# AegisIK/DistMLIP

Hardware: NVIDIA H100
Metric: atoms/sec (energy+forces) CHGNet a-Si r_cut=5A (higher is better)
Workload: dtype f32

## Files before the change

### distmlip_b200/csrc/kernels.cu

```cuda
#include "final_tail.cuh"
#include "kernels.cuh"
#include "wgmma.cuh"

#include <algorithm>

namespace b2m {

__device__ __forceinline__ float sigm(float x) {
  float e, r;
  asm("ex2.approx.ftz.f32 %0, %1;" : "=f"(e) : "f"(x * -1.4426950408889634f));
  asm("rcp.approx.ftz.f32 %0, %1;" : "=f"(r) : "f"(1.f + e));
  return r;
}
__device__ __forceinline__ float silu_f(float x) { return x * sigm(x); }
__device__ __forceinline__ float dsilu_f(float x) {
  float s = sigm(x);
  return s * (1.f + x * (1.f - s));
}

__device__ __forceinline__ uint32_t smem_u32(const void* p) { return (uint32_t)__cvta_generic_to_shared(p); }
__device__ __forceinline__ void mbar_init(uint64_t* bar, uint32_t count) {
  asm volatile("mbarrier.init.shared::cta.b64 [%0], %1;" ::"r"(smem_u32(bar)), "r"(count) : "memory");
}
__device__ __forceinline__ void fence_barrier_init() {
// ... 225 lines not shown
}
__global__ void k_dsilu_mul(int64_t n, const float* __restrict__ pre, float* __restrict__ g) {
  const int64_t i = blockIdx.x * (int64_t)blockDim.x + threadIdx.x;
  if (i < n) g[i] *= dsilu_f(pre[i]);
}
void launch_silu(cudaStream_t st, int64_t n, const float* pre, float* out) {
  launch(k_silu, cdiv(n, 256), 256, 0, st, n, pre, out);
}
void launch_dsilu_mul(cudaStream_t st, int64_t n, const float* pre, float* g) {
  launch(k_dsilu_mul, cdiv(n, 256), 256, 0, st, n, pre, g);
}
void launch_zero_rows(cudaStream_t st, float* p, int64_t nfloats) {
  if (nfloats > 0) B2M_CK(cudaMemsetAsync(p, 0, nfloats * sizeof(float), st));
}

constexpr int LDE = 136;

struct EdgeRow {
  int src, dst, bond;
  float d;
};
__device__ __forceinline__ EdgeRow edge_row(const AtomConvArgs& a, int64_t e, bool has_row) {
  EdgeRow r{-1, -1, -1, 1.f};
  if (has_row && e < a.E) {
    r.src = a.e_src[e];
    r.dst = a.e_dst[e];
    r.bond = a.e_bond[e];
    r.d = a.e_vec[e].w;
  }
  return r;
}
template <int ROWS>
__device__ __forceinline__ void issue_gather(const AtomConvArgs& a, int64_t t, const EdgeRow& row, int lr, float* buf,
                                             uint64_t* bar, int* s_src, int* s_dst, int* s_bond, float* s_d) {
  if (lr == 0) mbar_expect_tx(bar, (uint32_t)min((int64_t)ROWS, a.E - t * ROWS) * 512u);
  if (lr < ROWS) {
    if (s_src != nullptr) s_src[lr] = row.src;
    s_dst[lr] = row.dst;
    s_bond[lr] = row.bond;
    s_d[lr] = row.d;
    if (row.src >= 0) bulk_g2s(buf + lr * LDE, a.Aproj + (size_t)row.src * D2, 512u, bar);
  }
}
template <int ROWS>
__device__ __forceinline__ void radial_rows(const AtomConvArgs& a, const float* s_d, int nvalid, float* be_s, float* be8,
                                            float* dbe_s, float* dbe8) {
  const int r = threadIdx.x % ROWS, half = (threadIdx.x / ROWS) & 1;
  const float d = s_d[r];
  const int k0 = half ? 5 : 0, k1 = half ? 9 : 5;
  for (int k = k0; k < k1; k++) {
    float be = 0.f, dbe = 0.f;
    if (r < nvalid) rbf_env_k(d, a.rp.freq[k], a.rp, be, dbe);
    *(k < 8 ? be_s + r * 8 + k : be8 + r) = be;
    if (dbe_s != nullptr) *(k < 8 ? dbe_s + r * 8 + k : dbe8 + r) = dbe;
  }
}
__device__ __forceinline__ float2 ld_f2(const float* p) { return *reinterpret_cast<const float2*>(p); }
__device__ __forceinline__ void st_f2(float* p, float x, float y) { *reinterpret_cast<float2*>(p) = make_float2(x, y); }

__device__ __forceinline__ constexpr int fq(int ii, int j) { return 4 * (j >> 1) + 2 * ii + (j & 1); }

__device__ __forceinline__ void radial_mma(const Map& m, int h, const float* x_s, const float* img, float (&d)[32]) {
  const float2 u = ld_f2(x_s + m.row(2 * h) * 8 + m.cb), v = ld_f2(x_s + m.row(2 * h + 1) * 8 + m.cb);
  const float x[1][4] = {{u.x, v.x, u.y, v.y}};
  uint32_t b = s_u32(img);
  asm volatile("" : "+r"(b));
  wg_mma64(x, b, b + 512u * 4u, 0, false, d);
}

template <int R>
__device__ __forceinline__ void first_layer_half(const AtomConvArgs& a, const Map& m, int h, const float* tile,
                                                 const int* s_dst, const int* s_bond, const float* be_s,
                                                 const float* be8, const float* rad, int nvalid,
                                                 float (&acc)[R][AC]) {
  const int c0 = 64 * m.branch + m.cb;
  float2 cv[2][AC / 2], qv[2][AC / 2];
  float b8[2];
  bool viaQ[2], ok[2];
#pragma unroll
  for (int ii = 0; ii < 2; ii++) {
    const int r = m.row(2 * h + ii);
    const int dst = s_dst[r], bond = s_bond[r];
    ok[ii] = r < nvalid;
    viaQ[ii] = a.Qproj != nullptr && bond >= 0;
    const float* cp = a.Cproj + (size_t)max(dst, 0) * D2 + c0;
#pragma unroll
    for (int jj = 0; jj < AC / 2; jj++) cv[ii][jj] = dst >= 0 ? __ldg(reinterpret_cast<const float2*>(cp + 8 * jj)) : make_float2(0.f, 0.f);
    if (viaQ[ii]) {
      const float* qp = a.Qproj + (size_t)bond * D2 + c0;
#pragma unroll
      for (int jj = 0; jj < AC / 2; jj++) qv[ii][jj] = __ldg(reinterpret_cast<const float2*>(qp + 8 * jj));
    } else {
#pragma unroll
      for (int jj = 0; jj < AC / 2; jj++) qv[ii][jj] = make_float2(0.f, 0.f);
    }
    b8[ii] = be8[r];
  }
  float d[32];
  radial_mma(m, h, be_s, rad + ATOM_RAD_M + 1024 * m.branch, d);
#pragma unroll
  for (int j = 0; j < AC; j++) {
    const float m8 = rad[ATOM_RAD_M8 + 64 * m.branch + m.col(j)];
#pragma unroll
    for (int ii = 0; ii < 2; ii++) {
      const int r = m.row(2 * h + ii);
      const float x = tile[r * LDE + 64 * m.branch + m.col(j)];
      const float2 c2 = cv[ii][j >> 1], q2 = qv[ii][j >> 1];
      const float t = viaQ[ii] ? ((j & 1) ? q2.y : q2.x) : fmaf(b8[ii], m8, d[fq(ii, j)]);
      acc[2 * h + ii][j] = ok[ii] ? x + ((j & 1) ? c2.y : c2.x) + t : 0.f;
    }
  }
}

template <int R>
__device__ __forceinline__ void wg_mm64_acc(const float (&x)[R][AC], int h, const float* Bcan, float (&acc)[R][AC]) {
  float v[8][4];
#pragma unroll
  for (int ks = 0; ks < 8; ks++) {
    v[ks][0] = x[2 * h][2 * ks], v[ks][1] = x[2 * h + 1][2 * ks];
    v[ks][2] = x[2 * h][2 * ks + 1], v[ks][3] = x[2 * h + 1][2 * ks + 1];
  }
  const uint32_t b_hi = s_u32(Bcan);
  float d[32];
  wg_mma64(v, b_hi, b_hi + 4096u * 4u, 0, false, d);
#pragma unroll
  for (int q = 0; q < 32; q++) acc[2 * h + ((q >> 1) & 1)][2 * (q >> 2) + (q & 1)] = d[q];
}

__device__ __forceinline__ float quad_row_sum(const float (&v)[AR]) {
  const int l = threadIdx.x & 3;
  const bool b0 = l & 1, b1 = l & 2;
  float w[2];
#pragma unroll
  for (int h = 0; h < 2; h++)
    w[h] = (b0 ? v[2 * h + 1] : v[2 * h]) + __shfl_xor_sync(0xffffffffu, b0 ? v[2 * h] : v[2 * h + 1], 1);
  return (b1 ? w[1] : w[0]) + __shfl_xor_sync(0xffffffffu, b1 ? w[0] : w[1], 2);
}

__device__ __forceinline__ void red_add_v4(float* p, float4 v) {
  asm volatile("red.global.add.v4.f32 [%0], {%1, %2, %3, %4};" ::"l"(p), "f"(v.x), "f"(v.y), "f"(v.z), "f"(v.w)
               : "memory");
}

__device__ __forceinline__ void seg_add(float* out, int width, int col, int k, const float4& v, int& cur, float4& sum) {
  if (k != cur) {
    if (cur >= 0) red_add_v4(out + (size_t)cur * width + col, sum);
    cur = k;
    sum = make_float4(0.f, 0.f, 0.f, 0.f);
  }
  if (k >= 0) sum.x += v.x, sum.y += v.y, sum.z += v.z, sum.w += v.w;
}

template <int LPR, int ROWS = TM, int NTH = NT>
__device__ __forceinline__ void scatter_rows(const float* tile, const int* key0, float* out0, const int* key1,
                                             float* out1, const int* gidx, float* gat, const int* sidx = nullptr,
                                             float* sto = nullptr) {
  constexpr int R = ROWS * LPR / NTH, W = 4 * LPR, B = 8;
  static_assert(R % B == 0 && B % 4 == 0, "batches of B rows, their indices read as int4");
  const int t = threadIdx.x % NTH, q = t % LPR, r0 = t / LPR * R;
  float4 s0 = make_float4(0.f, 0.f, 0.f, 0.f), s1 = s0;
  int c0 = -1, c1 = -1;
#pragma unroll
  for (int b = 0; b < R; b += B) {
    float4 v[B];
    int k0[B], k1[B], kg[B], ks[B];
#pragma unroll
    for (int i = 0; i < B; i++) v[i] = *reinterpret_cast<const float4*>(tile + (r0 + b + i) * LDE + 4 * q);
    auto ld_idx = [&](const int* idx, bool on, int(&k)[B]) {
#pragma unroll
      for (int i = 0; i < B; i += 4) {
        const int4 x = on ? *reinterpret_cast<const int4*>(idx + r0 + b + i) : make_int4(-1, -1, -1, -1);
        k[i] = x.x, k[i + 1] = x.y, k[i + 2] = x.z, k[i + 3] = x.w;
      }
    };
    ld_idx(key0, out0 != nullptr, k0);
    ld_idx(key1, out1 != nullptr, k1);
    ld_idx(gidx, gat != nullptr, kg);
    ld_idx(sidx, sto != nullptr, ks);
#pragma unroll
    for (int i = 0; i < B; i++) {
      if (ks[i] >= 0) *reinterpret_cast<float4*>(sto + (size_t)ks[i] * W + 4 * q) = v[i];
      if (kg[i] >= 0) red_add_v4(gat + (size_t)kg[i] * W + 4 * q, v[i]);
      seg_add(out0, W, 4 * q, k0[i], v[i], c0, s0);
      seg_add(out1, W, 4 * q, k1[i], v[i], c1, s1);
    }
  }
  if (c0 >= 0) red_add_v4(out0 + (size_t)c0 * W + 4 * q, s0);
  if (c1 >= 0) red_add_v4(out1 + (size_t)c1 * W + 4 * q, s1);
}

constexpr int TW = 64;
constexpr int WGF = 3, NTF = 128 * WGF;
struct AtomSmemFwd {
  static constexpr int kTile = 32;
  static constexpr int kW = kTile + WGF * TW * LDE;
  static constexpr int kRad = kW + 16384;
  static constexpr int kBe = kRad + ATOM_RAD;
  static constexpr int kBe8 = kBe + WGF * TW * 8;
  static constexpr int kB2 = kBe8 + WGF * TW;
  static constexpr int kD = kB2 + 128;
  static constexpr int kIdx = kD + WGF * TW;
  static constexpr int kTotal = kIdx + 2 * WGF * TW;
  static constexpr size_t bytes = (size_t)kTotal * 4;
};
static_assert(AtomSmemFwd::bytes <= 232448, "atom-conv forward shared memory");
static_assert(AtomSmemFwd::kW % 4 == 0 && AtomSmemFwd::kRad % 4 == 0 && AtomSmemFwd::kBe % 4 == 0 &&
                  AtomSmemFwd::kIdx % 4 == 0,
              "16-byte aligned images, radial rows and index slots");

__device__ __forceinline__ void wg_sync(int w) { asm volatile("bar.sync %0, 128;" ::"r"(1 + w) : "memory"); }

__global__ void __launch_bounds__(NTF, 1) k_atomconv_fwd(const AtomConvArgs a) {
  extern __shared__ __align__(128) float smem[];
  const int tid = threadIdx.x, w = tid >> 7, lr = tid & 127;
  uint64_t* mbar = reinterpret_cast<uint64_t*>(smem) + w;
  const float* Wsm = smem + AtomSmemFwd::kW;
  const float* rad = smem + AtomSmemFwd::kRad;
  const float* b2s = smem + AtomSmemFwd::kB2;
  float* tile = smem + AtomSmemFwd::kTile + w * TW * LDE;
  float* be_s = smem + AtomSmemFwd::kBe + w * TW * 8;
  float* be8 = smem + AtomSmemFwd::kBe8 + w * TW;
  float* s_d = smem + AtomSmemFwd::kD + w * TW;
  int* s_dst = reinterpret_cast<int*>(smem + AtomSmemFwd::kIdx) + w * TW;
  int* s_bond = reinterpret_cast<int*>(smem + AtomSmemFwd::kIdx) + (WGF + w) * TW;

  const int64_t ntiles = (a.E + TW - 1) / TW, first = WGF * (int64_t)blockIdx.x + w, step = WGF * (int64_t)gridDim.x;
  if (tid == 0) {
    for (int i = 0; i < WGF; i++) mbar_init(reinterpret_cast<uint64_t*>(smem) + i, 1);
    fence_barrier_init();
  }
  EdgeRow nxt = edge_row(a, first * TW + lr, lr < TW);
  stage_w<NTF>(smem + AtomSmemFwd::kW, a.W2can, 4096);
  stage_w<NTF>(smem + AtomSmemFwd::kRad, a.radial, ATOM_RAD / 4);
  if (tid < 128) smem[AtomSmemFwd::kB2 + tid] = a.b2[tid];
  __syncthreads();
  if (first < ntiles)
    issue_gather<TW>(a, first, nxt, lr, tile, mbar, nullptr, s_dst, s_bond, s_d);
  nxt = edge_row(a, (first + step) * TW + lr, lr < TW);

  const Map m;
  Map mL = m, mG = m;
  mL.branch = 0;
  mG.branch = 1;
  int it = 0;
  for (int64_t t = first; t < ntiles; t += step, it++) {
    const int nvalid = (int)min((int64_t)TW, a.E - t * TW);
    wg_sync(w);
    radial_rows<TW>(a, s_d, nvalid, be_s, be8, nullptr, nullptr);
    mbar_wait(mbar, (uint32_t)it & 1u);
    wg_sync(w);
    float L[2][AC];
    first_layer_half(a, mL, 0, tile, s_dst, s_bond, be_s, be8, rad, nvalid, L);
#pragma unroll
    for (int ii = 0; ii < 2; ii++)
#pragma unroll
      for (int j = 0; j < AC; j++) L[ii][j] = silu_f(L[ii][j]);
    wg_mm64_acc(L, 0, Wsm, L);
#pragma unroll
    for (int ii = 0; ii < 2; ii++)
#pragma unroll
      for (int j = 0; j < AC; j++) L[ii][j] = silu_f(L[ii][j] + b2s[m.col(j)]);
    float G[2][AC];
    first_layer_half(a, mG, 0, tile, s_dst, s_bond, be_s, be8, rad, nvalid, G);
#pragma unroll
    for (int ii = 0; ii < 2; ii++)
#pragma unroll
      for (int j = 0; j < AC; j++) G[ii][j] = silu_f(G[ii][j]);
    wg_mm64_acc(G, 0, Wsm + 8192, G);
    float wab[32];
    radial_mma(m, 0, be_s, rad + ATOM_RAD_WAB, wab);
#pragma unroll
    for (int ii = 0; ii < 2; ii++) {
      const int r = m.row(ii);
      const float b8 = be8[r];
      float mv[AC];
#pragma unroll
      for (int j = 0; j < AC; j++) {
        const float g = sigm(G[ii][j] + b2s[64 + m.col(j)]) * fmaf(b8, rad[ATOM_RAD_WAB8 + m.col(j)], wab[fq(ii, j)]);
        mv[j] = L[ii][j] * g;
      }
#pragma unroll
      for (int jj = 0; jj < AC / 2; jj++) st_f2(tile + r * LDE + m.col(2 * jj), mv[2 * jj], mv[2 * jj + 1]);
    }
    wg_sync(w);
    scatter_rows<16, TW, 128>(tile, s_dst, a.agg, nullptr, nullptr, nullptr, nullptr);
    fence_proxy_async_smem();
    wg_sync(w);
    if (t + step < ntiles) {
      issue_gather<TW>(a, t + step, nxt, lr, tile, mbar, nullptr, s_dst, s_bond, s_d);
      nxt = edge_row(a, (t + 2 * step) * TW + lr, lr < TW);
    }
  }
}

void launch_atomconv_fwd(cudaStream_t st, const AtomConvArgs& a, int num_sms) {
  if (a.E <= 0) return;
  static PerDeviceOnce attr;
  if (auto once_ = attr.first(); once_) {
    B2M_CK(cudaFuncSetAttribute(k_atomconv_fwd, cudaFuncAttributeMaxDynamicSharedMemorySize, (int)AtomSmemFwd::bytes));
  }
  launch(k_atomconv_fwd, std::min(cdiv(cdiv(a.E, TW), WGF), num_sms), NTF, AtomSmemFwd::bytes, st, a);
}

struct AtomSmemBwd {
  static constexpr int kBuf = 32;
  static constexpr int kW = kBuf + 2 * TM * LDE;
  static constexpr int kRad = kW + 16384;
  static constexpr int kBe = kRad + ATOM_RAD;
  static constexpr int kDbe = kBe + TM * 8;
  static constexpr int kBe8 = kDbe + TM * 8;
  static constexpr int kDbe8 = kBe8 + TM;
  static constexpr int kB2 = kDbe8 + TM;
  static constexpr int kD = kB2 + 128;
  static constexpr int kIdx = kD + 2 * TM;
  static constexpr int kTotal = kIdx + 6 * TM;
  static constexpr size_t bytes = (size_t)kTotal * 4;
};
static_assert(AtomSmemBwd::bytes <= 232448, "atom-conv backward shared memory");
static_assert(AtomSmemBwd::kW % 4 == 0 && AtomSmemBwd::kRad % 4 == 0 && AtomSmemBwd::kBe % 4 == 0 &&
                  AtomSmemBwd::kDbe % 4 == 0,
              "16-byte aligned images and radial rows");

__global__ void __launch_bounds__(NT, 1) k_atomconv_bwd(const AtomConvArgs a) {
  extern __shared__ __align__(128) float smem[];
  uint64_t* gbar = reinterpret_cast<uint64_t*>(smem);
  uint64_t* wbar = gbar + 2;
  float* Wsm = smem + AtomSmemBwd::kW;
  float* rad_base = smem + AtomSmemBwd::kRad;
  float* be_s = smem + AtomSmemBwd::kBe;
  float* dbe_s = smem + AtomSmemBwd::kDbe;
  float* be8 = smem + AtomSmemBwd::kBe8;
  float* dbe8 = smem + AtomSmemBwd::kDbe8;
  float* b2s = smem + AtomSmemBwd::kB2;

  const int tid = threadIdx.x;
  const int64_t ntiles = (a.E + TM - 1) / TM, step = gridDim.x;
  const bool useQ = a.Qproj != nullptr;
  auto buf_of = [&](int s) { return smem + AtomSmemBwd::kBuf + s * TM * LDE; };
  auto d_of = [&](int s) { return smem + AtomSmemBwd::kD + s * TM; };
  auto src_of = [&](int s) { return reinterpret_cast<int*>(smem + AtomSmemBwd::kIdx) + s * TM; };
  auto dst_of = [&](int s) { return reinterpret_cast<int*>(smem + AtomSmemBwd::kIdx) + (2 + s) * TM; };
  auto bond_of = [&](int s) { return reinterpret_cast<int*>(smem + AtomSmemBwd::kIdx) + (4 + s) * TM; };

  if (tid == 0) {
    mbar_init(&gbar[0], 1);
    mbar_init(&gbar[1], 1);
    mbar_init(wbar, 1);
    fence_barrier_init();
  }
  EdgeRow nxt = edge_row(a, (int64_t)blockIdx.x * TM + tid, threadIdx.x < TM);
  stage_w(rad_base, a.radial, ATOM_RAD / 4);
  if (tid < 128) b2s[tid] = a.b2[tid];
  __syncthreads();
  if (tid == 0) bulk_g2s_image(Wsm, a.W2can, 16384 * 4, wbar);
  issue_gather<TM>(a, blockIdx.x, nxt, tid, buf_of(0), &gbar[0], src_of(0), dst_of(0), bond_of(0), d_of(0));
  nxt = edge_row(a, ((int64_t)blockIdx.x + step) * TM + tid, threadIdx.x < TM);
  uint32_t wpar = 0;

  const Map m;
  const int c0 = 64 * m.branch;
  int it = 0;
  for (int64_t t = blockIdx.x; t < ntiles; t += step, it++) {
    float* rad = rad_base;
    asm volatile("" : "+l"(rad));
    const int s = it & 1;
    float* tileP = buf_of(s);
    float* tileH = buf_of(s ^ 1);
    const int* s_src = src_of(s);
    const int* s_dst = dst_of(s);
    const int* s_bond = bond_of(s);
    const int64_t e0 = t * TM;
    const int nvalid = (int)min((int64_t)TM, a.E - e0);
    __syncthreads();
    radial_rows<TM>(a, d_of(s), nvalid, be_s, be8, dbe_s, dbe8);
    mbar_wait(&gbar[s], stage_parity(it));
    mbar_wait(wbar, wpar);
    wpar ^= 1;
    __syncthreads();
    float acc[AR][AC];
#pragma unroll
    for (int h = 0; h < 2; h++) {
      first_layer_half(a, m, h, tileP, s_dst, s_bond, be_s, be8, rad, nvalid, acc);
#pragma unroll
      for (int ii = 0; ii < 2; ii++)
#pragma unroll
        for (int jj = 0; jj < AC / 2; jj++) {
          float* p = tileP + m.row(2 * h + ii) * LDE + c0 + m.col(2 * jj);
          float& x0 = acc[2 * h + ii][2 * jj];
          float& x1 = acc[2 * h + ii][2 * jj + 1];
          st_f2(p, x0, x1);
          x0 = silu_f(x0);
          x1 = silu_f(x1);
        }
      wg_mm64_acc(acc, h, Wsm + m.branch * 8192, acc);
#pragma unroll
      for (int ii = 0; ii < 2; ii++)
#pragma unroll
        for (int jj = 0; jj < AC / 2; jj++) {
          const float u0 = acc[2 * h + ii][2 * jj] + b2s[m.branch * 64 + m.col(2 * jj)];
          const float u1 = acc[2 * h + ii][2 * jj + 1] + b2s[m.branch * 64 + m.col(2 * jj + 1)];
          st_f2(tileH + m.row(2 * h + ii) * LDE + c0 + m.col(2 * jj), m.branch == 0 ? u0 : sigm(u0),
                m.branch == 0 ? u1 : sigm(u1));
        }
    }
    __syncthreads();
    if (tid == 0) bulk_g2s_image(Wsm, a.W2Tcan, 16384 * 4, wbar);
    float sd[AR];
#pragma unroll
    for (int h = 0; h < 2; h++) {
      int dst[2];
      float2 gm2[2][AC / 2];
#pragma unroll
      for (int ii = 0; ii < 2; ii++) {
        dst[ii] = s_dst[m.row(2 * h + ii)];
        const float* gp = a.gagg + (size_t)max(dst[ii], 0) * D + m.cb;
#pragma unroll
        for (int jj = 0; jj < AC / 2; jj++)
          gm2[ii][jj] = dst[ii] >= 0 ? __ldg(reinterpret_cast<const float2*>(gp + 8 * jj)) : make_float2(0.f, 0.f);
      }
      float w[32];
      radial_mma(m, h, be_s, rad + ATOM_RAD_WAB, w);
#pragma unroll
      for (int ii = 0; ii < 2; ii++) {
        const int i = 2 * h + ii;
        const int r = m.row(i);
        const float b8 = be8[r];
#pragma unroll
        for (int jj = 0; jj < AC / 2; jj++) {
          const float2 ow2 = ld_f2(tileH + r * LDE + c0 + m.col(2 * jj));
          const float2 pt2 = ld_f2(tileH + r * LDE + (64 - c0) + m.col(2 * jj));
          const float2 wk2 = ld_f2(rad + ATOM_RAD_WAB8 + m.col(2 * jj));
#pragma unroll
          for (int e = 0; e < 2; e++) {
            const int j = 2 * jj + e;
            const float x = e ? ow2.y : ow2.x;
            const float pt = e ? pt2.y : pt2.x;
            const float gm = e ? gm2[ii][jj].y : gm2[ii][jj].x;
            const float wab = fmaf(b8, e ? wk2.y : wk2.x, w[fq(ii, j)]);
            float g = 0.f, gwv = 0.f;
            if (dst[ii] >= 0) {
              if (m.branch == 0) {
                const float sg = sigm(x);
                const float oL = x * sg;
                gwv = gm * oL * pt;
                g = gm * pt * wab * (sg * (1.f + x * (1.f - sg)));
              } else {
                const float oL = silu_f(pt);
                g = gm * oL * wab * x * (1.f - x);
              }
            }
            acc[i][j] = g;
            w[fq(ii, j)] = gwv;
          }
        }
      }
      sd[2 * h] = sd[2 * h + 1] = 0.f;
      if (m.branch == 0) {
        float dw[32];
        radial_mma(m, h, dbe_s, rad + ATOM_RAD_WAB, dw);
#pragma unroll
        for (int ii = 0; ii < 2; ii++) {
          const float db8 = dbe8[m.row(2 * h + ii)];
#pragma unroll
          for (int j = 0; j < AC; j++)
            sd[2 * h + ii] = fmaf(w[fq(ii, j)], fmaf(db8, rad[ATOM_RAD_WAB8 + m.col(j)], dw[fq(ii, j)]), sd[2 * h + ii]);
        }
      }
      if (h == 0) mbar_wait(wbar, wpar);
      wg_mm64_acc(acc, h, Wsm + m.branch * 8192, acc);
#pragma unroll
      for (int ii = 0; ii < 2; ii++)
#pragma unroll
        for (int jj = 0; jj < AC / 2; jj++) {
          float* p = tileP + m.row(2 * h + ii) * LDE + c0 + m.col(2 * jj);
          const float2 pre = ld_f2(p);
          float& x0 = acc[2 * h + ii][2 * jj];
          float& x1 = acc[2 * h + ii][2 * jj + 1];
          x0 *= dsilu_f(pre.x);
          x1 *= dsilu_f(pre.y);
          st_f2(p, x0, x1);
        }
      float dm[32];
      radial_mma(m, h, dbe_s, rad + ATOM_RAD_M + 1024 * m.branch, dm);
#pragma unroll
      for (int ii = 0; ii < 2; ii++) {
        const int r = m.row(2 * h + ii);
        const float db8 = dbe8[r];
        float s = 0.f;
#pragma unroll
        for (int jj = 0; jj < AC / 2; jj++) {
          const float2 mk = ld_f2(rad + ATOM_RAD_M8 + c0 + m.col(2 * jj));
          s = fmaf(acc[2 * h + ii][2 * jj], fmaf(db8, mk.x, dm[fq(ii, 2 * jj)]), s);
          s = fmaf(acc[2 * h + ii][2 * jj + 1], fmaf(db8, mk.y, dm[fq(ii, 2 * jj + 1)]), s);
        }
        if (r < nvalid && !(useQ && s_bond[r] >= 0)) sd[2 * h + ii] += s;
      }
    }
    wpar ^= 1;
    fence_proxy_async_smem();
    __syncthreads();
    if (t + step < ntiles) {
      if (tid == 0) bulk_g2s_image(Wsm, a.W2can, 16384 * 4, wbar);
      issue_gather<TM>(a, t + step, nxt, tid, tileH, &gbar[s ^ 1], src_of(s ^ 1), dst_of(s ^ 1), bond_of(s ^ 1), d_of(s ^ 1));
      nxt = edge_row(a, (t + 2 * step) * TM + tid, threadIdx.x < TM);
    }
    {
      const float v = quad_row_sum(sd);
      const int r = m.row(tid & 3);
      if (m.branch == 1) be8[r] = v;
      __syncthreads();
      if (m.branch == 0 && r < nvalid) a.gd[e0 + r] += v + be8[r];
    }
    scatter_rows<32>(tileP, s_dst, a.gA != nullptr ? a.gC : nullptr, nullptr, nullptr, s_src, a.gA, s_bond,
                     useQ ? a.gQ : nullptr);
  }
}

void launch_atomconv_bwd(cudaStream_t st, const AtomConvArgs& a, int num_sms) {
  if (a.E <= 0) return;
  static PerDeviceOnce attr;
  if (auto once_ = attr.first(); once_) {
    B2M_CK(cudaFuncSetAttribute(k_atomconv_bwd, cudaFuncAttributeMaxDynamicSharedMemorySize, (int)AtomSmemBwd::bytes));
  }
  launch(k_atomconv_bwd, std::min(cdiv(a.E, TM), num_sms), NT, AtomSmemBwd::bytes, st, a);
}

struct LineSmem {
  static constexpr int kBuf = 32;
  static constexpr int kW = kBuf + 2 * TM * LDE;
  static constexpr int kB2 = kW + 16384;
  static constexpr int kIdx = kB2 + 128;
  static constexpr int kTotal = kIdx + 6 * TM;
  static constexpr size_t bytes = (size_t)kTotal * 4;
};
static_assert(LineSmem::bytes <= 232448, "line-graph shared memory");

struct LineSm {
  float* smem;
  __device__ __forceinline__ uint64_t* hbar() const { return reinterpret_cast<uint64_t*>(smem); }
  __device__ __forceinline__ uint64_t* abar() const { return hbar() + 2; }
  __device__ __forceinline__ uint64_t* wbar() const { return hbar() + 4; }
  __device__ __forceinline__ float* buf(int s) const { return smem + LineSmem::kBuf + s * TM * LDE; }
  __device__ __forceinline__ float* W() const { return smem + LineSmem::kW; }
  __device__ __forceinline__ float* b2() const { return smem + LineSmem::kB2; }
  __device__ __forceinline__ int* idx(int s, int k) const {
    return reinterpret_cast<int*>(smem + LineSmem::kIdx) + (2 * k + s) * TM;
  }
};

struct AngleIdx {
  int a, b, c;
};
__device__ __forceinline__ AngleIdx angle_idx(const LineArgs& a, int64_t r) {
  AngleIdx x{-1, -1, -1};
  if (threadIdx.x < TM && r < a.A) {
    x.a = a.a_in[r];
    x.b = a.a_out[r];
    x.c = a.a_ctr[r];
  }
  return x;
}
__device__ __forceinline__ void line_issue_ha(const LineArgs& a, const LineSm& sm, int64_t t, const AngleIdx& x,
                                             float* buf, int s) {
  const int tid = threadIdx.x;
  if (tid == 0) mbar_expect_tx(&sm.hbar()[s], (uint32_t)min((int64_t)TM, a.A - t * TM) * 512u);
  if (tid < TM) {
    sm.idx(s, 0)[tid] = x.a;
    sm.idx(s, 1)[tid] = x.b;
    sm.idx(s, 2)[tid] = x.c;
    if (x.a >= 0) bulk_g2s(buf + tid * LDE, a.Ha + (size_t)x.a * D2, 512u, &sm.hbar()[s]);
  }
}
__device__ __forceinline__ void line_issue_ang(const LineArgs& a, const LineSm& sm, int64_t t, float* buf, int s) {
  const int tid = threadIdx.x;
  const int nvalid = (int)min((int64_t)TM, a.A - t * TM);
  if (tid == 0) mbar_expect_tx(&sm.abar()[s], (uint32_t)nvalid * 256u);
  if (tid < nvalid) bulk_g2s(buf + tid * LDE + 64, a.ang + (size_t)(t * TM + tid) * D, 256u, &sm.abar()[s]);
}
__device__ __forceinline__ AngleIdx line_prologue(const LineArgs& a, const LineSm& sm) {
  const int tid = threadIdx.x;
  if (tid == 0) {
    for (int i = 0; i < 5; i++) mbar_init(&sm.hbar()[i], 1);
    fence_barrier_init();
  }
  AngleIdx x = angle_idx(a, (int64_t)blockIdx.x * TM + tid);
  if (tid < 128) sm.b2()[tid] = a.b2 ? a.b2[tid] : 0.f;
  __syncthreads();
  if (tid == 0) bulk_g2s_image(sm.W(), a.Wgcan, 16384 * 4, sm.wbar());
  line_issue_ha(a, sm, blockIdx.x, x, sm.buf(0), 0);
  line_issue_ang(a, sm, blockIdx.x, sm.buf(1), 0);
  return angle_idx(a, ((int64_t)blockIdx.x + gridDim.x) * TM + tid);
}

__device__ __forceinline__ void line_first_layer(const LineArgs& a, const Map& m, const float* P, const int* s_b,
                                                 const int* s_c, int nvalid, float (&acc)[AR][AC]) {
  const int c0 = 64 * m.branch + m.cb;
#pragma unroll
  for (int i = 0; i < AR; i++) {
    const int r = m.row(i);
    const bool ok = r < nvalid;
    const float* hb = a.Hb + (size_t)(ok ? s_b[r] : 0) * D2 + c0;
    const float* xc = a.Xc + (size_t)(ok ? s_c[r] : 0) * D2 + c0;
    float2 hv[AC / 2], xv[AC / 2];
#pragma unroll
    for (int jj = 0; jj < AC / 2; jj++) {
      hv[jj] = ok ? __ldg(reinterpret_cast<const float2*>(hb + 8 * jj)) : make_float2(0.f, 0.f);
      xv[jj] = ok ? __ldg(reinterpret_cast<const float2*>(xc + 8 * jj)) : make_float2(0.f, 0.f);
    }
#pragma unroll
    for (int jj = 0; jj < AC / 2; jj++) {
      const float2 ha = ok ? ld_f2(P + r * LDE + c0 + 8 * jj) : make_float2(0.f, 0.f);
      float& x0 = acc[i][2 * jj];
      float& x1 = acc[i][2 * jj + 1];
      x0 = ok ? ha.x + x0 + hv[jj].x + xv[jj].x : 0.f;
      x1 = ok ? ha.y + x1 + hv[jj].y + xv[jj].y : 0.f;
    }
  }
}

__device__ __forceinline__ void red_add_v2(float* p, float x, float y) {
  asm volatile("red.global.add.v2.f32 [%0], {%1, %2};" ::"l"(p), "f"(x), "f"(y) : "memory");
}

template <bool HIDDEN>
__global__ void __launch_bounds__(NT, 1) k_line_fwd(const LineArgs a) {
  extern __shared__ __align__(128) float smem[];
  const LineSm sm{smem};
  const float* b2s = sm.b2();
  const int tid = threadIdx.x;
  const int64_t ntiles = (a.A + TM - 1) / TM, step = gridDim.x;
  AngleIdx nxt = line_prologue(a, sm);
  uint32_t wpar = 0;

  int it = 0;
  for (int64_t t = blockIdx.x; t < ntiles; t += step, it++) {
    const int s = it & 1;
    float* P = sm.buf(s);
    float* Q = sm.buf(s ^ 1);
    const int* s_b = sm.idx(s, 1);
    const int* s_c = sm.idx(s, 2);
    const int64_t r0 = t * TM;
    const int nvalid = (int)min((int64_t)TM, a.A - r0);
    const bool more = t + step < ntiles;
    const Map m;
    float acc[AR][AC];
    mbar_wait(&sm.abar()[s], stage_parity(it));
    mbar_wait(sm.wbar(), wpar);
    if (HIDDEN) wpar ^= 1;
    gemm64(Q, LDE, 64, sm.W() + m.branch * 8192, acc);
    fence_proxy_async_smem();
    __syncthreads();
    if (more) {
      line_issue_ha(a, sm, t + step, nxt, Q, s ^ 1);
      nxt = angle_idx(a, (t + 2 * step) * TM + tid);
    }
    if (HIDDEN && tid == 0) bulk_g2s_image(sm.W(), a.W2can, 16384 * 4, sm.wbar());
    mbar_wait(&sm.hbar()[s], stage_parity(it));
    line_first_layer(a, m, P, s_b, s_c, nvalid, acc);
#pragma unroll
    for (int i = 0; i < AR; i++)
#pragma unroll
      for (int j = 0; j < AC; j++) acc[i][j] = HIDDEN || m.branch == 0 ? silu_f(acc[i][j]) : sigm(acc[i][j]);
    if (HIDDEN) {
      mbar_wait(sm.wbar(), wpar);
      wpar ^= 1;
      wg_mm64_acc(acc, 0, sm.W() + m.branch * 8192, acc);
      wg_mm64_acc(acc, 1, sm.W() + m.branch * 8192, acc);
#pragma unroll
      for (int i = 0; i < AR; i++)
#pragma unroll
        for (int j = 0; j < AC; j++) {
          const float u = acc[i][j] + b2s[m.branch * 64 + m.col(j)];
          acc[i][j] = m.branch == 0 ? silu_f(u) : sigm(u);
        }
    }
    fence_proxy_async_smem();
    __syncthreads();
    if (more) {
      line_issue_ang(a, sm, t + step, P, s ^ 1);
      if (HIDDEN && tid == 0) bulk_g2s_image(sm.W(), a.Wgcan, 16384 * 4, sm.wbar());
    }
    if (m.branch == 1) {
#pragma unroll
      for (int i = 0; i < AR; i++)
#pragma unroll
        for (int jj = 0; jj < AC / 2; jj++) st_f2(P + m.row(i) * LDE + m.col(2 * jj), acc[i][2 * jj], acc[i][2 * jj + 1]);
    }
    __syncthreads();
    if (m.branch == 0) {
#pragma unroll
      for (int i = 0; i < AR; i++) {
        const int r = m.row(i);
        if (HIDDEN) {
#pragma unroll
          for (int jj = 0; jj < AC / 2; jj++) {
            float* p = P + r * LDE + m.col(2 * jj);
            const float2 g = ld_f2(p);
            st_f2(p, acc[i][2 * jj] * g.x, acc[i][2 * jj + 1] * g.y);
          }
        } else if (r < nvalid) {
          const float* ang = a.ang + (size_t)(r0 + r) * D;
          float* out = a.ang_out + (size_t)(r0 + r) * D;
          float2 av[AC / 2];
#pragma unroll
          for (int jj = 0; jj < AC / 2; jj++) av[jj] = __ldg(reinterpret_cast<const float2*>(ang + m.col(2 * jj)));
#pragma unroll
          for (int jj = 0; jj < AC / 2; jj++) {
            const int c = m.col(2 * jj);
            const float2 g = ld_f2(P + r * LDE + c);
            st_f2(out + c, av[jj].x + acc[i][2 * jj] * g.x, av[jj].y + acc[i][2 * jj + 1] * g.y);
          }
        }
      }
    }
    if (HIDDEN) {
      __syncthreads();
      scatter_rows<16>(P, s_b, a.aggB, nullptr, nullptr, nullptr, nullptr);
    }
  }
}

template <bool HIDDEN>
__global__ void __launch_bounds__(NT, 1) k_line_bwd(const LineArgs a) {
  extern __shared__ __align__(128) float smem[];
  const LineSm sm{smem};
  const float* b2s = sm.b2();
  const int tid = threadIdx.x;
  const int64_t ntiles = (a.A + TM - 1) / TM, step = gridDim.x;
  AngleIdx nxt = line_prologue(a, sm);
  uint32_t wpar = 0;

  int it = 0;
  for (int64_t t = blockIdx.x; t < ntiles; t += step, it++) {
    const int s = it & 1;
    float* P = sm.buf(s);
    float* H = sm.buf(s ^ 1);
    const int* s_a = sm.idx(s, 0);
    const int* s_b = sm.idx(s, 1);
    const int* s_c = sm.idx(s, 2);
    const int64_t r0 = t * TM;
    const int nvalid = (int)min((int64_t)TM, a.A - r0);
    const bool more = t + step < ntiles;
    const Map m;
    float acc[AR][AC];
    mbar_wait(&sm.abar()[s], stage_parity(it));
    mbar_wait(sm.wbar(), wpar);
    wpar ^= 1;
    gemm64(H, LDE, 64, sm.W() + m.branch * 8192, acc);
    __syncthreads();
    if (tid == 0) bulk_g2s_image(sm.W(), HIDDEN ? a.W2can : a.WgTcan, 16384 * 4, sm.wbar());
    mbar_wait(&sm.hbar()[s], stage_parity(it));
    line_first_layer(a, m, P, s_b, s_c, nvalid, acc);
    if (HIDDEN) {
#pragma unroll
      for (int i = 0; i < AR; i++)
#pragma unroll
        for (int jj = 0; jj < AC / 2; jj++) {
          float& x0 = acc[i][2 * jj];
          float& x1 = acc[i][2 * jj + 1];
          st_f2(P + m.row(i) * LDE + m.branch * 64 + m.col(2 * jj), x0, x1);
          x0 = silu_f(x0);
          x1 = silu_f(x1);
        }
      mbar_wait(sm.wbar(), wpar);
      wpar ^= 1;
    }
#pragma unroll
    for (int h = 0; h < 2; h++) {
      if (HIDDEN) wg_mm64_acc(acc, h, sm.W() + m.branch * 8192, acc);
#pragma unroll
      for (int ii = 0; ii < 2; ii++)
#pragma unroll
        for (int jj = 0; jj < AC / 2; jj++) {
          const int i = 2 * h + ii;
          const float u0 = HIDDEN ? acc[i][2 * jj] + b2s[m.branch * 64 + m.col(2 * jj)] : acc[i][2 * jj];
          const float u1 = HIDDEN ? acc[i][2 * jj + 1] + b2s[m.branch * 64 + m.col(2 * jj + 1)] : acc[i][2 * jj + 1];
          st_f2(H + m.row(i) * LDE + m.branch * 64 + m.col(2 * jj), m.branch == 0 ? u0 : sigm(u0),
                m.branch == 0 ? u1 : sigm(u1));
        }
    }
    __syncthreads();
    if (HIDDEN && tid == 0) bulk_g2s_image(sm.W(), a.W2Tcan, 16384 * 4, sm.wbar());
#pragma unroll
    for (int h = 0; h < 2; h++) {
      bool ok[2];
      float2 gm2[2][AC / 2];
#pragma unroll
      for (int ii = 0; ii < 2; ii++) {
        const int r = m.row(2 * h + ii);
        ok[ii] = r < nvalid;
        const float* gsrc =
            HIDDEN ? a.gaggB + (size_t)(ok[ii] ? s_b[r] : 0) * D : a.gang + (size_t)(r0 + (ok[ii] ? r : 0)) * D;
#pragma unroll
        for (int jj = 0; jj < AC / 2; jj++)
          gm2[ii][jj] = ok[ii] ? *reinterpret_cast<const float2*>(gsrc + m.col(2 * jj)) : make_float2(0.f, 0.f);
      }
#pragma unroll
      for (int ii = 0; ii < 2; ii++) {
        const int i = 2 * h + ii;
        const int r = m.row(i);
#pragma unroll
        for (int j = 0; j < AC; j++) {
          const float2 ow2 = ld_f2(H + r * LDE + m.branch * 64 + m.col(j & ~1));
          const float2 pt2 = ld_f2(H + r * LDE + (1 - m.branch) * 64 + m.col(j & ~1));
          const float x = (j & 1) ? ow2.y : ow2.x;
          const float pt = (j & 1) ? pt2.y : pt2.x;
          float g = 0.f;
          if (ok[ii]) {
            const float gm = (j & 1) ? gm2[ii][j >> 1].y : gm2[ii][j >> 1].x;
            if (m.branch == 0) {
              const float sg = sigm(x);
              g = gm * pt * (sg * (1.f + x * (1.f - sg)));
            } else {
              const float oL = silu_f(pt);
              g = gm * oL * x * (1.f - x);
            }
          }
          acc[i][j] = g;
        }
      }
      if (HIDDEN) {
        if (h == 0) mbar_wait(sm.wbar(), wpar);
        wg_mm64_acc(acc, h, sm.W() + m.branch * 8192, acc);
      }
#pragma unroll
      for (int ii = 0; ii < 2; ii++)
#pragma unroll
// ... 377 lines not shown
```

Baseline: 2.380 million.

## Restructure atom-conv backward into independent per-warpgroup tiles with resident weights

The atom-conv backward kernel now runs two independent warpgroups per block, each owning its own smaller edge tile, instead of the whole block cooperating on one large tile with block-wide barriers. Both W2 and W2^T stay resident in shared memory, which removes the per-tile bulk reloads of the weight image and the waits on that barrier. Each warpgroup computes both the L and G branches itself, and the cross-branch exchange goes through registers and shuffles rather than a second shared tile. In exchange, the gather is no longer double-buffered: it is issued only after the scatter finishes, so overlap between load and compute now comes only from the other warpgroup. Register pressure per thread also rises.

```diff
diff --git a/distmlip_b200/csrc/kernels.cu b/distmlip_b200/csrc/kernels.cu
--- a/distmlip_b200/csrc/kernels.cu
+++ b/distmlip_b200/csrc/kernels.cu
@@ -551,217 +551,200 @@
   launch(k_atomconv_fwd, std::min(cdiv(cdiv(a.E, TW), WGF), num_sms), NTF, AtomSmemFwd::bytes, st, a);
 }
 
+constexpr int WGB = 2, NTB = 128 * WGB;
 struct AtomSmemBwd {
-  static constexpr int kBuf = 32;
-  static constexpr int kW = kBuf + 2 * TM * LDE;
-  static constexpr int kRad = kW + 16384;
+  static constexpr int kTile = 32;
+  static constexpr int kW = kTile + WGB * TW * LDE;
+  static constexpr int kWT = kW + 16384;
+  static constexpr int kRad = kWT + 16384;
   static constexpr int kBe = kRad + ATOM_RAD;
-  static constexpr int kDbe = kBe + TM * 8;
-  static constexpr int kBe8 = kDbe + TM * 8;
-  static constexpr int kDbe8 = kBe8 + TM;
-  static constexpr int kB2 = kDbe8 + TM;
+  static constexpr int kDbe = kBe + WGB * TW * 8;
+  static constexpr int kBe8 = kDbe + WGB * TW * 8;
+  static constexpr int kDbe8 = kBe8 + WGB * TW;
+  static constexpr int kB2 = kDbe8 + WGB * TW;
   static constexpr int kD = kB2 + 128;
-  static constexpr int kIdx = kD + 2 * TM;
-  static constexpr int kTotal = kIdx + 6 * TM;
+  static constexpr int kIdx = kD + WGB * TW;
+  static constexpr int kTotal = kIdx + 3 * WGB * TW;
   static constexpr size_t bytes = (size_t)kTotal * 4;
 };
 static_assert(AtomSmemBwd::bytes <= 232448, "atom-conv backward shared memory");
-static_assert(AtomSmemBwd::kW % 4 == 0 && AtomSmemBwd::kRad % 4 == 0 && AtomSmemBwd::kBe % 4 == 0 &&
-                  AtomSmemBwd::kDbe % 4 == 0,
-              "16-byte aligned images and radial rows");
-
-__global__ void __launch_bounds__(NT, 1) k_atomconv_bwd(const AtomConvArgs a) {
+static_assert(AtomSmemBwd::kW % 4 == 0 && AtomSmemBwd::kWT % 4 == 0 && AtomSmemBwd::kRad % 4 == 0 &&
+                  AtomSmemBwd::kBe % 4 == 0 && AtomSmemBwd::kDbe % 4 == 0 && AtomSmemBwd::kIdx % 4 == 0,
+              "16-byte aligned images, radial rows and index slots");
+
+__global__ void __launch_bounds__(NTB, 1) k_atomconv_bwd(const AtomConvArgs a) {
   extern __shared__ __align__(128) float smem[];
-  uint64_t* gbar = reinterpret_cast<uint64_t*>(smem);
-  uint64_t* wbar = gbar + 2;
-  float* Wsm = smem + AtomSmemBwd::kW;
-  float* rad_base = smem + AtomSmemBwd::kRad;
-  float* be_s = smem + AtomSmemBwd::kBe;
-  float* dbe_s = smem + AtomSmemBwd::kDbe;
-  float* be8 = smem + AtomSmemBwd::kBe8;
-  float* dbe8 = smem + AtomSmemBwd::kDbe8;
-  float* b2s = smem + AtomSmemBwd::kB2;
-
-  const int tid = threadIdx.x;
-  const int64_t ntiles = (a.E + TM - 1) / TM, step = gridDim.x;
+  const int tid = threadIdx.x, w = tid >> 7, lr = tid & 127;
+  uint64_t* mbar = reinterpret_cast<uint64_t*>(smem) + w;
+  const float* W2s = smem + AtomSmemBwd::kW;
+  const float* W2Ts = smem + AtomSmemBwd::kWT;
+  const float* rad_base = smem + AtomSmemBwd::kRad;
+  const float* b2s = smem + AtomSmemBwd::kB2;
+  float* P = smem + AtomSmemBwd::kTile + w * TW * LDE;
+  float* be_s = smem + AtomSmemBwd::kBe + w * TW * 8;
+  float* dbe_s = smem + AtomSmemBwd::kDbe + w * TW * 8;
+  float* be8 = smem + AtomSmemBwd::kBe8 + w * TW;
+  float* dbe8 = smem + AtomSmemBwd::kDbe8 + w * TW;
+  float* s_d = smem + AtomSmemBwd::kD + w * TW;
+  int* s_src = reinterpret_cast<int*>(smem + AtomSmemBwd::kIdx) + w * TW;
+  int* s_dst = reinterpret_cast<int*>(smem + AtomSmemBwd::kIdx) + (WGB + w) * TW;
+  int* s_bond = reinterpret_cast<int*>(smem + AtomSmemBwd::kIdx) + (2 * WGB + w) * TW;
+
+  const int64_t ntiles = (a.E + TW - 1) / TW, first = WGB * (int64_t)blockIdx.x + w, step = WGB * (int64_t)gridDim.x;
   const bool useQ = a.Qproj != nullptr;
-  auto buf_of = [&](int s) { return smem + AtomSmemBwd::kBuf + s * TM * LDE; };
-  auto d_of = [&](int s) { return smem + AtomSmemBwd::kD + s * TM; };
-  auto src_of = [&](int s) { return reinterpret_cast<int*>(smem + AtomSmemBwd::kIdx) + s * TM; };
-  auto dst_of = [&](int s) { return reinterpret_cast<int*>(smem + AtomSmemBwd::kIdx) + (2 + s) * TM; };
-  auto bond_of = [&](int s) { return reinterpret_cast<int*>(smem + AtomSmemBwd::kIdx) + (4 + s) * TM; };
-
   if (tid == 0) {
-    mbar_init(&gbar[0], 1);
-    mbar_init(&gbar[1], 1);
-    mbar_init(wbar, 1);
+    for (int i = 0; i < WGB; i++) mbar_init(reinterpret_cast<uint64_t*>(smem) + i, 1);
     fence_barrier_init();
   }
-  EdgeRow nxt = edge_row(a, (int64_t)blockIdx.x * TM + tid, threadIdx.x < TM);
-  stage_w(rad_base, a.radial, ATOM_RAD / 4);
-  if (tid < 128) b2s[tid] = a.b2[tid];
+  EdgeRow nxt = edge_row(a, first * TW + lr, lr < TW);
+  stage_w<NTB>(smem + AtomSmemBwd::kW, a.W2can, 4096);
+  stage_w<NTB>(smem + AtomSmemBwd::kWT, a.W2Tcan, 4096);
+  stage_w<NTB>(smem + AtomSmemBwd::kRad, a.radial, ATOM_RAD / 4);
+  if (tid < 128) smem[AtomSmemBwd::kB2 + tid] = a.b2[tid];
   __syncthreads();
-  if (tid == 0) bulk_g2s_image(Wsm, a.W2can, 16384 * 4, wbar);
-  issue_gather<TM>(a, blockIdx.x, nxt, tid, buf_of(0), &gbar[0], src_of(0), dst_of(0), bond_of(0), d_of(0));
-  nxt = edge_row(a, ((int64_t)blockIdx.x + step) * TM + tid, threadIdx.x < TM);
-  uint32_t wpar = 0;
+  if (first < ntiles)
+    issue_gather<TW>(a, first, nxt, lr, P, mbar, s_src, s_dst, s_bond, s_d);
+  nxt = edge_row(a, (first + step) * TW + lr, lr < TW);
 
   const Map m;
-  const int c0 = 64 * m.branch;
+  Map mL = m, mG = m;
+  mL.branch = 0;
+  mG.branch = 1;
   int it = 0;
-  for (int64_t t = blockIdx.x; t < ntiles; t += step, it++) {
-    float* rad = rad_base;
+  for (int64_t t = first; t < ntiles; t += step, it++) {
+    const float* rad = rad_base;
     asm volatile("" : "+l"(rad));
-    const int s = it & 1;
-    float* tileP = buf_of(s);
-    float* tileH = buf_of(s ^ 1);
-    const int* s_src = src_of(s);
-    const int* s_dst = dst_of(s);
-    const int* s_bond = bond_of(s);
-    const int64_t e0 = t * TM;
-    const int nvalid = (int)min((int64_t)TM, a.E - e0);
-    __syncthreads();
-    radial_rows<TM>(a, d_of(s), nvalid, be_s, be8, dbe_s, dbe8);
-    mbar_wait(&gbar[s], stage_parity(it));
-    mbar_wait(wbar, wpar);
-    wpar ^= 1;
-    __syncthreads();
-    float acc[AR][AC];
-#pragma unroll
-    for (int h = 0; h < 2; h++) {
-      first_layer_half(a, m, h, tileP, s_dst, s_bond, be_s, be8, rad, nvalid, acc);
+    const int64_t e0 = t * TW;
+    const int nvalid = (int)min((int64_t)TW, a.E - e0);
+    wg_sync(w);
+    radial_rows<TW>(a, s_d, nvalid, be_s, be8, dbe_s, dbe8);
+    mbar_wait(mbar, (uint32_t)it & 1u);
+    wg_sync(w);
+    float L[2][AC], G[2][AC];
+    auto recompute = [&](const Map& mb, float(&x)[2][AC]) {
+      first_layer_half(a, mb, 0, P, s_dst, s_bond, be_s, be8, rad, nvalid, x);
 #pragma unroll
       for (int ii = 0; ii < 2; ii++)
 #pragma unroll
         for (int jj = 0; jj < AC / 2; jj++) {
-          float* p = tileP + m.row(2 * h + ii) * LDE + c0 + m.col(2 * jj);
-          float& x0 = acc[2 * h + ii][2 * jj];
-          float& x1 = acc[2 * h + ii][2 * jj + 1];
-          st_f2(p, x0, x1);
+          float& x0 = x[ii][2 * jj];
+          float& x1 = x[ii][2 * jj + 1];
+          st_f2(P + m.row(ii) * LDE + 64 * mb.branch + m.col(2 * jj), x0, x1);
           x0 = silu_f(x0);
           x1 = silu_f(x1);
         }
-      wg_mm64_acc(acc, h, Wsm + m.branch * 8192, acc);
-#pragma unroll
-      for (int ii = 0; ii < 2; ii++)
-#pragma unroll
-        for (int jj = 0; jj < AC / 2; jj++) {
-          const float u0 = acc[2 * h + ii][2 * jj] + b2s[m.branch * 64 + m.col(2 * jj)];
-          const float u1 = acc[2 * h + ii][2 * jj + 1] + b2s[m.branch * 64 + m.col(2 * jj + 1)];
-          st_f2(tileH + m.row(2 * h + ii) * LDE + c0 + m.col(2 * jj), m.branch == 0 ? u0 : sigm(u0),
-                m.branch == 0 ? u1 : sigm(u1));
-        }
-    }
-    __syncthreads();
-    if (tid == 0) bulk_g2s_image(Wsm, a.W2Tcan, 16384 * 4, wbar);
-    float sd[AR];
-#pragma unroll
-    for (int h = 0; h < 2; h++) {
-      int dst[2];
-      float2 gm2[2][AC / 2];
-#pragma unroll
-      for (int ii = 0; ii < 2; ii++) {
-        dst[ii] = s_dst[m.row(2 * h + ii)];
-        const float* gp = a.gagg + (size_t)max(dst[ii], 0) * D + m.cb;
-#pragma unroll
-        for (int jj = 0; jj < AC / 2; jj++)
-          gm2[ii][jj] = dst[ii] >= 0 ? __ldg(reinterpret_cast<const float2*>(gp + 8 * jj)) : make_float2(0.f, 0.f);
-      }
-      float w[32];
-      radial_mma(m, h, be_s, rad + ATOM_RAD_WAB, w);
-#pragma unroll
-      for (int ii = 0; ii < 2; ii++) {
-        const int i = 2 * h + ii;
-        const int r = m.row(i);
-        const float b8 = be8[r];
-#pragma unroll
-        for (int jj = 0; jj < AC / 2; jj++) {
-          const float2 ow2 = ld_f2(tileH + r * LDE + c0 + m.col(2 * jj));
-          const float2 pt2 = ld_f2(tileH + r * LDE + (64 - c0) + m.col(2 * jj));
-          const float2 wk2 = ld_f2(rad + ATOM_RAD_WAB8 + m.col(2 * jj));
-#pragma unroll
-          for (int e = 0; e < 2; e++) {
-            const int j = 2 * jj + e;
-            const float x = e ? ow2.y : ow2.x;
-            const float pt = e ? pt2.y : pt2.x;
-            const float gm = e ? gm2[ii][jj].y : gm2[ii][jj].x;
-            const float wab = fmaf(b8, e ? wk2.y : wk2.x, w[fq(ii, j)]);
-            float g = 0.f, gwv = 0.f;
-            if (dst[ii] >= 0) {
-              if (m.branch == 0) {
-                const float sg = sigm(x);
-                const float oL = x * sg;
-                gwv = gm * oL * pt;
-                g = gm * pt * wab * (sg * (1.f + x * (1.f - sg)));
-              } else {
-                const float oL = silu_f(pt);
-                g = gm * oL * wab * x * (1.f - x);
-              }
-            }
-            acc[i][j] = g;
-            w[fq(ii, j)] = gwv;
+      wg_mm64_acc(x, 0, W2s + mb.branch * 8192, x);
+    };
+    recompute(mL, L);
+#pragma unroll
+    for (int ii = 0; ii < 2; ii++)
+#pragma unroll
+      for (int j = 0; j < AC; j++) L[ii][j] += b2s[m.col(j)];
+    recompute(mG, G);
+#pragma unroll
+    for (int ii = 0; ii < 2; ii++)
+#pragma unroll
+      for (int j = 0; j < AC; j++) G[ii][j] = sigm(G[ii][j] + b2s[64 + m.col(j)]);
+    int dst[2];
+    float2 gm2[2][AC / 2];
+#pragma unroll
+    for (int ii = 0; ii < 2; ii++) {
+      dst[ii] = s_dst[m.row(ii)];
+      const float* gp = a.gagg + (size_t)max(dst[ii], 0) * D + m.cb;
+#pragma unroll
+      for (int jj = 0; jj < AC / 2; jj++)
+        gm2[ii][jj] = dst[ii] >= 0 ? __ldg(reinterpret_cast<const float2*>(gp + 8 * jj)) : make_float2(0.f, 0.f);
+    }
+    float wv[32];
+    radial_mma(m, 0, be_s, rad + ATOM_RAD_WAB, wv);
+#pragma unroll
+    for (int ii = 0; ii < 2; ii++) {
+      const float b8 = be8[m.row(ii)];
+#pragma unroll
+      for (int jj = 0; jj < AC / 2; jj++) {
+        const float2 wk2 = ld_f2(rad + ATOM_RAD_WAB8 + m.col(2 * jj));
+#pragma unroll
+        for (int e = 0; e < 2; e++) {
+          const int j = 2 * jj + e;
+          const float u = L[ii][j], oG = G[ii][j];
+          const float gm = e ? gm2[ii][jj].y : gm2[ii][jj].x;
+          const float wab = fmaf(b8, e ? wk2.y : wk2.x, wv[fq(ii, j)]);
+          float gu = 0.f, gv = 0.f, gwv = 0.f;
+          if (dst[ii] >= 0) {
+            const float sg = sigm(u);
+            const float oL = u * sg;
+            gwv = gm * oL * oG;
+            gu = gm * oG * wab * (sg * (1.f + u * (1.f - sg)));
+            gv = gm * oL * wab * oG * (1.f - oG);
           }
+          L[ii][j] = gu;
+          G[ii][j] = gv;
+          wv[fq(ii, j)] = gwv;
         }
       }
-      sd[2 * h] = sd[2 * h + 1] = 0.f;
-      if (m.branch == 0) {
-        float dw[32];
-        radial_mma(m, h, dbe_s, rad + ATOM_RAD_WAB, dw);
-#pragma unroll
-        for (int ii = 0; ii < 2; ii++) {
-          const float db8 = dbe8[m.row(2 * h + ii)];
-#pragma unroll
-          for (int j = 0; j < AC; j++)
-            sd[2 * h + ii] = fmaf(w[fq(ii, j)], fmaf(db8, rad[ATOM_RAD_WAB8 + m.col(j)], dw[fq(ii, j)]), sd[2 * h + ii]);
-        }
+    }
+    float sd[AR];
+    {
+      float dw[32];
+      radial_mma(m, 0, dbe_s, rad + ATOM_RAD_WAB, dw);
+#pragma unroll
+      for (int ii = 0; ii < 2; ii++) {
+        const float db8 = dbe8[m.row(ii)];
+        float s = 0.f;
+#pragma unroll
+        for (int j = 0; j < AC; j++) s = fmaf(wv[fq(ii, j)], fmaf(db8, rad[ATOM_RAD_WAB8 + m.col(j)], dw[fq(ii, j)]), s);
+        sd[ii] = s;
+        sd[2 + ii] = 0.f;
       }
-      if (h == 0) mbar_wait(wbar, wpar);
-      wg_mm64_acc(acc, h, Wsm + m.branch * 8192, acc);
+    }
+    auto reverse = [&](const Map& mb, float(&x)[2][AC]) {
+      const int c0 = 64 * mb.branch;
+      wg_mm64_acc(x, 0, W2Ts + mb.branch * 8192, x);
 #pragma unroll
       for (int ii = 0; ii < 2; ii++)
 #pragma unroll
         for (int jj = 0; jj < AC / 2; jj++) {
-          float* p = tileP + m.row(2 * h + ii) * LDE + c0 + m.col(2 * jj);
+          float* p = P + m.row(ii) * LDE + c0 + m.col(2 * jj);
           const float2 pre = ld_f2(p);
-          float& x0 = acc[2 * h + ii][2 * jj];
-          float& x1 = acc[2 * h + ii][2 * jj + 1];
+          float& x0 = x[ii][2 * jj];
+          float& x1 = x[ii][2 * jj + 1];
           x0 *= dsilu_f(pre.x);
           x1 *= dsilu_f(pre.y);
           st_f2(p, x0, x1);
         }
       float dm[32];
-      radial_mma(m, h, dbe_s, rad + ATOM_RAD_M + 1024 * m.branch, dm);
+      radial_mma(m, 0, dbe_s, rad + ATOM_RAD_M + 1024 * mb.branch, dm);
 #pragma unroll
       for (int ii = 0; ii < 2; ii++) {
-        const int r = m.row(2 * h + ii);
+        const int r = m.row(ii);
         const float db8 = dbe8[r];
         float s = 0.f;
 #pragma unroll
         for (int jj = 0; jj < AC / 2; jj++) {
           const float2 mk = ld_f2(rad + ATOM_RAD_M8 + c0 + m.col(2 * jj));
-          s = fmaf(acc[2 * h + ii][2 * jj], fmaf(db8, mk.x, dm[fq(ii, 2 * jj)]), s);
-          s = fmaf(acc[2 * h + ii][2 * jj + 1], fmaf(db8, mk.y, dm[fq(ii, 2 * jj + 1)]), s);
+          s = fmaf(x[ii][2 * jj], fmaf(db8, mk.x, dm[fq(ii, 2 * jj)]), s);
+          s = fmaf(x[ii][2 * jj + 1], fmaf(db8, mk.y, dm[fq(ii, 2 * jj + 1)]), s);
         }
-        if (r < nvalid && !(useQ && s_bond[r] >= 0)) sd[2 * h + ii] += s;
+        if (r < nvalid && !(useQ && s_bond[r] >= 0)) sd[2 * mb.branch + ii] += s;
       }
-    }
-    wpar ^= 1;
-    fence_proxy_async_smem();
-    __syncthreads();
-    if (t + step < ntiles) {
-      if (tid == 0) bulk_g2s_image(Wsm, a.W2can, 16384 * 4, wbar);
-      issue_gather<TM>(a, t + step, nxt, tid, tileH, &gbar[s ^ 1], src_of(s ^ 1), dst_of(s ^ 1), bond_of(s ^ 1), d_of(s ^ 1));
-      nxt = edge_row(a, (t + 2 * step) * TM + tid, threadIdx.x < TM);
-    }
+    };
+    reverse(mL, L);
+    reverse(mG, G);
     {
       const float v = quad_row_sum(sd);
-      const int r = m.row(tid & 3);
-      if (m.branch == 1) be8[r] = v;
-      __syncthreads();
-      if (m.branch == 0 && r < nvalid) a.gd[e0 + r] += v + be8[r];
-    }
-    scatter_rows<32>(tileP, s_dst, a.gA != nullptr ? a.gC : nullptr, nullptr, nullptr, s_src, a.gA, s_bond,
-                     useQ ? a.gQ : nullptr);
+      const float v1 = __shfl_xor_sync(0xffffffffu, v, 2);
+      const int r = m.row(tid & 1);
+      if ((tid & 2) == 0 && r < nvalid) a.gd[e0 + r] += v + v1;
+    }
+    wg_sync(w);
+    scatter_rows<32, TW, 128>(P, s_dst, a.gA != nullptr ? a.gC : nullptr, nullptr, nullptr, s_src, a.gA, s_bond,
+                              useQ ? a.gQ : nullptr);
+    fence_proxy_async_smem();
+    wg_sync(w);
+    if (t + step < ntiles) {
+      issue_gather<TW>(a, t + step, nxt, lr, P, mbar, s_src, s_dst, s_bond, s_d);
+      nxt = edge_row(a, (t + 2 * step) * TW + lr, lr < TW);
+    }
   }
 }
 
@@ -771,7 +754,7 @@
   if (auto once_ = attr.first(); once_) {
     B2M_CK(cudaFuncSetAttribute(k_atomconv_bwd, cudaFuncAttributeMaxDynamicSharedMemorySize, (int)AtomSmemBwd::bytes));
   }
-  launch(k_atomconv_bwd, std::min(cdiv(a.E, TM), num_sms), NT, AtomSmemBwd::bytes, st, a);
+  launch(k_atomconv_bwd, std::min(cdiv(cdiv(a.E, TW), WGB), num_sms), NTB, AtomSmemBwd::bytes, st, a);
 }
 
 struct LineSmem {
```

Result: faster. 2.571 million, median of 6 (+8.0%).
